# Gadersd/stable-diffusion-xl-burn

Measured on NVIDIA H100. Metric: unet_sampler_steps_per_sec_1024x1024_bs1, higher is better.
Workload: dtype f16

## Files before the change

stable-diffusion-xl-burn_b200/csrc/attention.cu:

```cuda
#include <stdlib.h>

#include "common.cuh"
#include "kernels.h"

namespace sdxl {

static constexpr int kTileBytes = 128 * 128;
static constexpr int kKvStages = 3;
static constexpr int kConsumerWarps = 8;
static constexpr int kAttnThreads = kConsumerWarps * 32 + 32;
static constexpr int kAttnSmem = 1024  + kTileBytes + 2 * kKvStages * kTileBytes + 256;

__device__ __forceinline__ float ex2_approx(float x) {
  float y;
  asm("ex2.approx.ftz.f32 %0, %1;" : "=f"(y) : "f"(x));
  return y;
}
__device__ __forceinline__ uint32_t pack_half2(float a, float b) {
  __half2 t = __floats2half2_rn(a, b);
  return *reinterpret_cast<uint32_t*>(&t);
}

__device__ __forceinline__ void attn_key_block(float (&o)[32], float (&m)[2], float (&l)[2], uint32_t q_addr, const uint8_t* sK,
                                               const uint8_t* sV, uint64_t* kv_full, uint64_t* kv_empty, int j, int kb, int S,
                                               float sl2e, int lane) {
  const int st = j % kKvStages;
  mbar_wait_nocall(&kv_full[st], (j / kKvStages) & 1);
  float s[64];
  wg_fence();
  const uint32_t k_addr = smem_u32(sK + st * kTileBytes);
#pragma unroll
  for (int k = 0; k < 4; ++k) wgmma_ss_n128(s, wg_desc_sw128(q_addr + 32 * k), wg_desc_sw128(k_addr + 32 * k), k);
  wg_commit();
  wg_wait<0>();
  if (kb * 128 + 128 > S) {
#pragma unroll
    for (int jj = 0; jj < 16; ++jj)
#pragma unroll
      for (int e = 0; e < 2; ++e)
        if (kb * 128 + 8 * jj + 2 * (lane & 3) + e >= S) { s[4 * jj + e] = -INFINITY; s[4 * jj + 2 + e] = -INFINITY; }
  }
  uint32_t pa[32];
#pragma unroll
  for (int h = 0; h < 2; ++h) {
    float mx = -INFINITY;
#pragma unroll
    for (int jj = 0; jj < 16; ++jj) mx = fmaxf(mx, fmaxf(s[4 * jj + 2 * h], s[4 * jj + 2 * h + 1]));
    mx = fmaxf(mx, __shfl_xor_sync(0xffffffffu, mx, 1));
    mx = fmaxf(mx, __shfl_xor_sync(0xffffffffu, mx, 2));
    const float m_new = fmaxf(m[h], mx);
    const float alpha = ex2_approx((m[h] - m_new) * sl2e);
    const float mb = m_new * sl2e;
    float sum = 0.f;
#pragma unroll
    for (int jj = 0; jj < 16; ++jj) {
      const float p0 = ex2_approx(fmaf(s[4 * jj + 2 * h], sl2e, -mb));
      const float p1 = ex2_approx(fmaf(s[4 * jj + 2 * h + 1], sl2e, -mb));
      sum += p0 + p1;
      pa[4 * (jj >> 1) + 2 * (jj & 1) + h] = pack_half2(p0, p1);
    }
    l[h] = l[h] * alpha + sum;
    m[h] = m_new;
#pragma unroll
    for (int jj = 0; jj < 8; ++jj) { o[4 * jj + 2 * h] *= alpha; o[4 * jj + 2 * h + 1] *= alpha; }
  }
  wg_fence();
  const uint32_t v_addr = smem_u32(sV + st * kTileBytes);
#pragma unroll
  for (int kk = 0; kk < 8; ++kk)
    wgmma_rs_n64_tb(o, *reinterpret_cast<const uint32_t(*)[4]>(pa + 4 * kk), wg_desc_sw128(v_addr + 2048 * kk));
  wg_commit();
  wg_wait<0>();
  if (lane == 0) mbar_arrive(&kv_empty[st]);
}

struct IpSrc {
  const CUtensorMap* tk;
  const CUtensorMap* tv;
  int S, k_col0, v_col0;
  const float* scale;
  const float* mask;
};
__device__ __forceinline__ IpSrc ip_source(const AttnParams& p, int k) {
  if (k == 0) return {&p.tmKip, &p.tmVip, p.S_ip, p.k_ip_col0, p.v_ip_col0, p.ip_scale, p.ip_mask};
  const AttnIpSource& s = p.ip_src[k - 1];
  return {&s.tm, &s.tm, s.S, s.k_col0, s.v_col0, s.scale, s.mask};
}

template <bool kIp>
__global__ void __launch_bounds__(kAttnThreads, 1) attention_kernel(const __grid_constant__ AttnParams p) {
  extern __shared__ uint8_t smem_raw[];
  uint8_t* smem = reinterpret_cast<uint8_t*>((reinterpret_cast<uintptr_t>(smem_raw) + 1023) & ~uintptr_t(1023));
  uint8_t* sQ = smem;
  uint8_t* sK = sQ + kTileBytes;
  uint8_t* sV = sK + kKvStages * kTileBytes;
  uint64_t* bars = reinterpret_cast<uint64_t*>(sV + kKvStages * kTileBytes);
  uint64_t* q_full = bars;
  uint64_t* kv_full = q_full + 1;
  uint64_t* kv_empty = kv_full + kKvStages;

  const int warp = threadIdx.x >> 5, lane = threadIdx.x & 31;
  const int nblk = (p.S + 127) / 128;
  const int nqt = (p.T + 127) / 128;
  const int qt = blockIdx.x % nqt, head = (blockIdx.x / nqt) % p.n_head, b = blockIdx.x / (nqt * p.n_head);

  if (threadIdx.x == 0) {
    tma_prefetch_desc(&p.tmQ);
    tma_prefetch_desc(&p.tmK);
    tma_prefetch_desc(&p.tmV);
    if constexpr (kIp) {
      tma_prefetch_desc(&p.tmKip);
      tma_prefetch_desc(&p.tmVip);
      for (int k = 1; k < p.n_src; ++k) tma_prefetch_desc(&p.ip_src[k - 1].tm);
    }
    mbar_init(q_full, 1);
    for (int i = 0; i < kKvStages; ++i) { mbar_init(&kv_full[i], 1); mbar_init(&kv_empty[i], kConsumerWarps); }
    fence_barrier_init();
  }
  __syncthreads();
  griddep_wait();
  griddep_launch_dependents();

  if (warp == kConsumerWarps) {
    if (lane != 0) return;
    mbar_expect_tx(q_full, kTileBytes);
    tma_load_3d(sQ, &p.tmQ, q_full, p.q_col0 + head * 64, qt * 128, b);
    for (int j = 0; j < nblk; ++j) {
      const int st = j % kKvStages;
      mbar_wait_nocall(&kv_empty[st], ((j / kKvStages) & 1) ^ 1);
      mbar_expect_tx(&kv_full[st], 2 * kTileBytes);
      tma_load_3d(sK + st * kTileBytes, &p.tmK, &kv_full[st], p.k_col0 + head * 64, j * 128, b);
      tma_load_3d(sV + st * kTileBytes, &p.tmV, &kv_full[st], p.v_col0 + head * 64, j * 128, b);
    }
    if constexpr (kIp) {
      int j = nblk;
      for (int k = 0; k < p.n_src; ++k) {
        const IpSrc s = ip_source(p, k);
        const int nb = (s.S + 127) / 128;
        for (int kb = 0; kb < nb; ++kb, ++j) {
          const int st = j % kKvStages;
          mbar_wait_nocall(&kv_empty[st], ((j / kKvStages) & 1) ^ 1);
          mbar_expect_tx(&kv_full[st], 2 * kTileBytes);
          tma_load_3d(sK + st * kTileBytes, s.tk, &kv_full[st], s.k_col0 + head * 64, kb * 128, b);
          tma_load_3d(sV + st * kTileBytes, s.tv, &kv_full[st], s.v_col0 + head * 64, kb * 128, b);
        }
      }
    }
    return;
  }

  const int wg = warp >> 2;
  const float sl2e = p.scale_log2e;
  const uint32_t q_addr = smem_u32(sQ) + (uint32_t)wg * (64 * 128);
  float o[32];
#pragma unroll
  for (int i = 0; i < 32; ++i) o[i] = 0.f;
  float m[2] = {-INFINITY, -INFINITY}, l[2] = {0.f, 0.f};
  mbar_wait_nocall(q_full, 0);
  for (int j = 0; j < nblk; ++j) {
    const int st = j % kKvStages;
    mbar_wait_nocall(&kv_full[st], (j / kKvStages) & 1);
    float s[64];
    wg_fence();
    const uint32_t k_addr = smem_u32(sK + st * kTileBytes);
#pragma unroll
    for (int k = 0; k < 4; ++k) wgmma_ss_n128(s, wg_desc_sw128(q_addr + 32 * k), wg_desc_sw128(k_addr + 32 * k), k);
    wg_commit();
    wg_wait<0>();
    if (j * 128 + 128 > p.S) {
#pragma unroll
      for (int jj = 0; jj < 16; ++jj)
#pragma unroll
        for (int e = 0; e < 2; ++e)
          if (j * 128 + 8 * jj + 2 * (lane & 3) + e >= p.S) { s[4 * jj + e] = -INFINITY; s[4 * jj + 2 + e] = -INFINITY; }
    }
    uint32_t pa[32];
#pragma unroll
    for (int h = 0; h < 2; ++h) {
      float mx = -INFINITY;
#pragma unroll
      for (int jj = 0; jj < 16; ++jj) mx = fmaxf(mx, fmaxf(s[4 * jj + 2 * h], s[4 * jj + 2 * h + 1]));
      mx = fmaxf(mx, __shfl_xor_sync(0xffffffffu, mx, 1));
      mx = fmaxf(mx, __shfl_xor_sync(0xffffffffu, mx, 2));
      const float m_new = fmaxf(m[h], mx);
      const float alpha = ex2_approx((m[h] - m_new) * sl2e);
      const float mb = m_new * sl2e;
      float sum = 0.f;
#pragma unroll
      for (int jj = 0; jj < 16; ++jj) {
        const float p0 = ex2_approx(fmaf(s[4 * jj + 2 * h], sl2e, -mb));
        const float p1 = ex2_approx(fmaf(s[4 * jj + 2 * h + 1], sl2e, -mb));
        sum += p0 + p1;
        pa[4 * (jj >> 1) + 2 * (jj & 1) + h] = pack_half2(p0, p1);
      }
      l[h] = l[h] * alpha + sum;
      m[h] = m_new;
#pragma unroll
      for (int jj = 0; jj < 8; ++jj) { o[4 * jj + 2 * h] *= alpha; o[4 * jj + 2 * h + 1] *= alpha; }
    }
    wg_fence();
    const uint32_t v_addr = smem_u32(sV + st * kTileBytes);
#pragma unroll
    for (int kk = 0; kk < 8; ++kk)
      wgmma_rs_n64_tb(o, *reinterpret_cast<const uint32_t(*)[4]>(pa + 4 * kk), wg_desc_sw128(v_addr + 2048 * kk));
    wg_commit();
    wg_wait<0>();
    if (lane == 0) mbar_arrive(&kv_empty[st]);
  }
  const int r = wg * 64 + (warp & 3) * 16 + (lane >> 2);
  if constexpr (kIp) {
    float acc[32];
#pragma unroll
    for (int h = 0; h < 2; ++h) {
      float lt = l[h];
      lt += __shfl_xor_sync(0xffffffffu, lt, 1);
      lt += __shfl_xor_sync(0xffffffffu, lt, 2);
      const float inv = 1.0f / lt;
#pragma unroll
      for (int jj = 0; jj < 8; ++jj) {
        acc[4 * jj + 2 * h] = o[4 * jj + 2 * h] * inv;
        acc[4 * jj + 2 * h + 1] = o[4 * jj + 2 * h + 1] * inv;
      }
    }
    int j = nblk;
    for (int k = 0; k < p.n_src; ++k) {
#pragma unroll
      for (int h = 0; h < 2; ++h) { m[h] = -INFINITY; l[h] = 0.f; }
#pragma unroll
      for (int i = 0; i < 32; ++i) o[i] = 0.f;
      const int S = ip_source(p, k).S;
      for (int kb = 0; kb * 128 < S; ++kb, ++j) attn_key_block(o, m, l, q_addr, sK, sV, kv_full, kv_empty, j, kb, S, sl2e, lane);
      const IpSrc s = ip_source(p, k);
      const float sk = *s.scale;
#pragma unroll
      for (int h = 0; h < 2; ++h) {
        float lt = l[h];
        lt += __shfl_xor_sync(0xffffffffu, lt, 1);
        lt += __shfl_xor_sync(0xffffffffu, lt, 2);
        const float inv = 1.0f / lt;
        const int t = qt * 128 + r + 8 * h;
        const float w = (s.mask && t < p.T) ? sk * s.mask[t] : sk;
#pragma unroll
        for (int jj = 0; jj < 8; ++jj) {
          acc[4 * jj + 2 * h] = fmaf(w, o[4 * jj + 2 * h] * inv, acc[4 * jj + 2 * h]);
          acc[4 * jj + 2 * h + 1] = fmaf(w, o[4 * jj + 2 * h + 1] * inv, acc[4 * jj + 2 * h + 1]);
        }
      }
    }
#pragma unroll
    for (int h = 0; h < 2; ++h) {
      const int t = qt * 128 + r + 8 * h;
      if (t < p.T) {
        __half* out = p.out + ((size_t)b * p.T + t) * p.ldo + head * 64 + 2 * (lane & 3);
#pragma unroll
// ... 42 lines not shown
  out[i] = cubic_1d(row[0], row[1], row[2], row[3], ty);
}

int ip_mask_resize_launch(cudaStream_t st, const float* mask, int H, int W, int mh, int mw, int T, float* out) {
  if (H < 1 || W < 1 || mh < 1 || mw < 1 || T < 1) return 2002;
  ip_mask_resize_kernel<<<(T + 255) / 256, 256, 0, st>>>(mask, H, W, mh, mw, T, out);
  return (int)cudaGetLastError();
}

static bool g_attn_attr[2][64];
int attention_launch(cudaStream_t st, const AttnParams& p) {
  if (p.T < 1 || p.S < 1 || (p.ldo & 1)) return 2002;
  const bool ip = p.S_ip > 0;
  if (ip && (!p.ip_scale || p.n_src < 1 || p.n_src > ATTN_MAX_SRC)) return 2002;
  for (int k = 1; ip && k < p.n_src; ++k)
    if (p.ip_src[k - 1].S < 1 || !p.ip_src[k - 1].scale) return 2002;
  auto kernel = ip ? attention_kernel<true> : attention_kernel<false>;
  int r = smem_optin(kernel, kAttnSmem, g_attn_attr[ip]);
  if (r) return r;
  const long tiles = (long)p.B * p.n_head * ((p.T + 127) / 128);
  return launch_kernel(kernel, dim3((unsigned)tiles), dim3(kAttnThreads), (size_t)kAttnSmem, st, true, p);
}

}
```

stable-diffusion-xl-burn_b200/csrc/engine.cu:

```cuda
#include "engine_core.h"
#include "schedule.h"

#include <set>

extern "C" int sdxl_ctx_create(int device, void* cuda_stream, sdxl_ctx** out) {
  if (!out) return -1;
  *out = nullptr;
  int n = 0;
  if (cudaGetDeviceCount(&n) != cudaSuccess || n <= 0 || device >= n) {
    fprintf(stderr, "sdxl_b200: no CUDA device %d (this library has no CPU fallback)\n", device);
    return -2;
  }
  cudaDeviceProp prop;
  if (cudaGetDeviceProperties(&prop, device) != cudaSuccess) return -3;
  if (prop.major != 9 || prop.minor != 0) {
    fprintf(stderr, "sdxl_b200: device %d is sm_%d%d; this library contains sm_90a code only\n", device,
            prop.major, prop.minor);
    return -4;
  }
  if (cudaSetDevice(device) != cudaSuccess) return -5;
  sdxl_ctx* c = new sdxl_ctx();
  c->device = device;
  c->num_sms = prop.multiProcessorCount;
  if (cuda_stream) {
// ... 825 lines not shown
      if (&b == &s.blocks.back()) linear(s_ff, M, b.ff2, IGEMM_LINEAR, s_a16, 0, C, s_tok, C);
      else linear(s_ff, M, b.ff2, IGEMM_LINEAR, s_tok, 1, C, s_tok, C);
    }
    if (s.blocks.empty() && !err) {
      Op op{};
      op.kind = OP_CAST16;
      op.cs = {s_tok, (size_t)M * C, s_a16};
      P->ops.push_back(op);
    }
    linear(s_a16, M, s.proj_out, IGEMM_LINEAR, out, 1, C, x, C);
    return out;
  }
  void attn(const __half* qm, int q_pitch, int q_col0, const __half* kvm, int kv_pitch, int k_col0, int v_col0, int T,
            int S, int n_head, __half* out, int ldo, float sl2e, int B = 0) {
    if (err) return;
    if (!B) B = Bf;
    Op op{};
    op.kind = OP_ATTN;
    AttnParams& p = op.at;
    p.T = T; p.S = S; p.n_head = n_head; p.B = B;
    p.q_col0 = q_col0; p.k_col0 = k_col0; p.v_col0 = v_col0;
    p.out = out; p.ldo = ldo; p.scale_log2e = sl2e;
    if (!A->measure) {
      int r = make_tmap_rows(&p.tmQ, qm, T, B, q_pitch, q_pitch);
      if (!r) r = make_tmap_rows(&p.tmK, kvm, S, B, kv_pitch, kv_pitch);
      if (!r) p.tmV = p.tmK;
      if (r) { err = fail(c, r, "tensor map creation failed (attention)"); return; }
    }
    op.flops_exec = 4.0 * B * (double)((T + 127) / 128 * 128) * (double)((S + 127) / 128 * 128) * (n_head * 64);
    P->ops.push_back(op);
    add_flops(4.0 * B * T * (double)S * (n_head * 64));
  }
  void attn_ip(const __half* kvm, int kv_pitch, int k_col0, int v_col0, int S_ip, const float* scale, const float* mask) {
    if (err) return;
    AttnParams& p = P->ops.back().at;
    if (p.n_src == ATTN_MAX_SRC) { err = fail(c, 5022, "image prompt: more than %d image sources", ATTN_MAX_SRC); return; }
    CUtensorMap tm{};
    if (!A->measure)
      if (int r = make_tmap_rows(&tm, kvm, S_ip, Bf, kv_pitch, kv_pitch)) { err = fail(c, r, "tensor map creation failed (attention)"); return; }
    if (p.n_src == 0) {
      p.S_ip = S_ip; p.k_ip_col0 = k_col0; p.v_ip_col0 = v_col0; p.ip_scale = scale; p.ip_mask = mask;
      p.tmKip = p.tmVip = tm;
    } else {
      p.ip_src[p.n_src - 1] = {tm, S_ip, k_col0, v_col0, scale, mask};
    }
    p.n_src++;
    const int C = p.n_head * 64;
    P->ops.back().flops_exec += 4.0 * Bf * (double)((p.T + 127) / 128 * 128) * (double)((S_ip + 127) / 128 * 128) * C;
    add_flops(4.0 * Bf * p.T * (double)S_ip * C);
  }
};



static int build_plan_ops(sdxl_unet* u, Plan* P, Arena* A, int Bp) {
  sdxl_ctx* c = u->ctx;
  const sdxl_unet_cfg& g = u->cfg;
  UNetPlanBuilder B{{c, P, A, P->Bf}, u};
  B.Bp = Bp;
  P->ops.clear();
  P->block_names.clear();
  P->flops = 0;
  const int Bf = P->Bf, mc = g.model_channels, ted = 4 * mc;
  const int temb_total = u->temb_all.N;
  const int levels = g.n_levels;
  if ((P->h % (1 << (levels - 1))) || (P->w % (1 << (levels - 1)))) return fail(c, 5003, "latent %dx%d not divisible by %d", P->h, P->w, 1 << (levels - 1));

  P->x_in = B.buf<float>((size_t)P->Bx * latent_channels(g) * P->h * P->w);
  P->eps_ld = g.out_channels;
  P->eps = B.buf<float>((size_t)Bf * P->h * P->w * P->eps_ld);
  B.gn_partial = B.buf<float>(gn_scratch_floats(Bf, 32));
// ... 1535 lines not shown
}

extern "C" void sdxl_unet_destroy(sdxl_unet* u) {
  if (!u) return;
  cudaStreamSynchronize(u->ctx->stream);
  delete u;
}


extern "C" int sdxl_qkv_attention(sdxl_ctx* c, const sdxl_half* q, const sdxl_half* k, const sdxl_half* v, const sdxl_half* mask,
                                  int B, int T, int S, int C, int n_head, sdxl_half* out) {
  if (!c || !q || !k || !v || !out) return -1;
  if (n_head < 1 || C != n_head * 64) return fail(c, 5301, "sdxl_qkv_attention: head dim must be 64 (C=%d, n_head=%d)", C, n_head);
  if (mask) {
    KL(c, attention_small_launch(c->stream, (const __half*)q, C, 0, (const __half*)k, (const __half*)v, C, 0, 0, B, T, S, n_head,
                                 (const __half*)mask, 0, (__half*)out, C));
    return 0;
  }
  AttnParams p{};
  p.T = T; p.S = S; p.n_head = n_head; p.B = B;
  p.q_col0 = p.k_col0 = p.v_col0 = 0;
  p.out = (__half*)out; p.ldo = C;
  p.scale_log2e = (float)(1.4426950408889634 / sqrt(64.0));
  int r = make_tmap_rows(&p.tmQ, (const __half*)q, T, B, C, C);
  if (!r) r = make_tmap_rows(&p.tmK, (const __half*)k, S, B, C, C);
  if (!r) r = make_tmap_rows(&p.tmV, (const __half*)v, S, B, C, C);
  if (r) return fail(c, r, "tensor map creation failed");
  KL(c, attention_launch(c->stream, p));
  return 0;
}

extern "C" int sdxl_op_ip_attention(sdxl_ctx* c, const sdxl_half* q, const sdxl_half* k, const sdxl_half* v, const sdxl_half* k_ip,
                                    const sdxl_half* v_ip, int B, int T, int S, int S_ip, int C, int n_head, float scale, sdxl_half* out) {
  if (!c || !q || !k || !v || !k_ip || !v_ip || !out) return -1;
  if (n_head < 1 || C != n_head * 64) return fail(c, 5302, "sdxl_op_ip_attention: head dim must be 64 (C=%d, n_head=%d)", C, n_head);
  if (B < 1 || S_ip < 1) return fail(c, 5303, "sdxl_op_ip_attention: B = %d and S_ip = %d must be >= 1", B, S_ip);
  CU(c, cudaSetDevice(c->device));
  TmpBufs tmp(c->stream);
  float* s = tmp.get<float>(sizeof(float));
  if (!s) return fail(c, 5304, "temporary allocation failed");
  CU(c, cudaMemcpyAsync(s, &scale, sizeof(float), cudaMemcpyHostToDevice, c->stream));
  AttnParams p{};
  p.T = T; p.S = S; p.n_head = n_head; p.B = B;
  p.out = (__half*)out; p.ldo = C;
  p.scale_log2e = (float)(1.4426950408889634 / sqrt(64.0));
  p.S_ip = S_ip; p.ip_scale = s; p.n_src = 1;
  int r = make_tmap_rows(&p.tmQ, (const __half*)q, T, B, C, C);
  if (!r) r = make_tmap_rows(&p.tmK, (const __half*)k, S, B, C, C);
  if (!r) r = make_tmap_rows(&p.tmV, (const __half*)v, S, B, C, C);
  if (!r) r = make_tmap_rows(&p.tmKip, (const __half*)k_ip, S_ip, B, C, C);
  if (!r) r = make_tmap_rows(&p.tmVip, (const __half*)v_ip, S_ip, B, C, C);
  if (r) return fail(c, r, "tensor map creation failed");
  KL(c, attention_launch(c->stream, p));
  CU(c, cudaStreamSynchronize(c->stream));
  return 0;
}

extern "C" int sdxl_op_linear(sdxl_ctx* c, const sdxl_half* x, const sdxl_half* w, const sdxl_half* bias, const float* residual,
                              int M, int K, int N, int geglu, int out_f16, void* out) {
  if (!c || !x || !w || !out) return -1;
  if (K % 8) return fail(c, 5310, "sdxl_op_linear: K must be a multiple of 8");
  TmpBufs T(c->stream);
  const int Kpad = (K + 63) / 64 * 64;
  int gbn = 0;
  if (geglu) {
    gbn = geglu_bn_for(N / 2);
    if (!gbn || (N & 1)) return fail(c, 5311, "sdxl_op_linear: GEGLU width not tileable");
  }
  __half* wt = T.get<__half>((size_t)N * Kpad * 2);
  float* b32 = bias ? T.get<float>((size_t)N * 4) : nullptr;
  if (!wt || (bias && !b32)) return fail(c, 5312, "temporary allocation failed");
  KL(c, transpose_linear_launch(c->stream, (const __half*)w, K, N, wt, Kpad, 0, gbn));
  if (bias) KL(c, bias_to_f32_launch(c->stream, (const __half*)bias, N, b32, gbn, 0));
  const IgemmOperands o{(const __half*)x, 1, 1, M, K, K, nullptr, 0, 0, 0, 0, 0, wt, N, Kpad};
// ... 64 lines not shown
```

stable-diffusion-xl-burn_b200/csrc/igemm.cu:

```cuda
#include "common.cuh"
#include "kernels.h"

#include <stdio.h>
#include <stdlib.h>

namespace sdxl {

static constexpr int kTileM = 128;
static constexpr int kBlockK = 64;
static constexpr int kABytes = kTileM * kBlockK * 2;
static constexpr int kConsumerWarps = 8;
static constexpr int kThreads = 128 + kConsumerWarps * 32;

__device__ __forceinline__ size_t out_pixel(const IgemmParams& p, int tb, int th, int tw, int r, bool& ok, int& bb) {
  const int wt = r % p.Wt, ht = (r / p.Wt) % p.Ht, bt = r / (p.Wt * p.Ht);
  bb = tb * p.Bt + bt;
  const int hh = th * p.Ht + ht, ww = tw * p.Wt + wt;
  ok = (bb < p.Bn) && (hh < p.H) && (ww < p.W);
  return ok ? ((size_t)bb * p.H + hh) * (size_t)p.opix_row + (size_t)ww * p.opix_w + p.opix_off : 0;
}

__device__ __forceinline__ void store2(const IgemmParams& p, size_t off, float x0, float x1, bool two, bool vec) {
  if (p.out_f32) {
    float* o = reinterpret_cast<float*>(p.out) + off;
// ... 194 lines not shown
  if (r != CUDA_SUCCESS) {
    fprintf(stderr, "sdxl_b200: cuTensorMapEncodeTiled failed (%d) rank=%d dims=[%llu,%llu,%llu,%llu] box=[%u,%u,%u,%u]\n",
            (int)r, rank, (unsigned long long)dims[0], (unsigned long long)(rank > 1 ? dims[1] : 0),
            (unsigned long long)(rank > 2 ? dims[2] : 0), (unsigned long long)(rank > 3 ? dims[3] : 0), box[0],
            rank > 1 ? box[1] : 0, rank > 2 ? box[2] : 0, rank > 3 ? box[3] : 0);
    return 1002;
  }
  return 0;
}

int make_tmap_act(CUtensorMap* tm, const __half* base, int Bn, int H, int W, int C, int pitch, int Wt, int Ht,
                  int Bt) {
  uint64_t dims[4] = {(uint64_t)C, (uint64_t)W, (uint64_t)H, (uint64_t)Bn};
  uint64_t str[3] = {(uint64_t)pitch * 2, (uint64_t)W * pitch * 2, (uint64_t)H * W * pitch * 2};
  uint32_t box[4] = {64, (uint32_t)Wt, (uint32_t)Ht, (uint32_t)Bt};
  return encode(tm, base, 4, dims, str, box);
}
int make_tmap_wgt(CUtensorMap* tm, const __half* base, int N, int K, int BN) {
  uint64_t dims[2] = {(uint64_t)K, (uint64_t)N};
  uint64_t str[1] = {(uint64_t)K * 2};
  uint32_t box[2] = {64, (uint32_t)BN};
  return encode(tm, base, 2, dims, str, box);
}
int make_tmap_rows(CUtensorMap* tm, const __half* base, int rows_per_batch, int nbatch, int cols, int pitch) {
  uint64_t dims[3] = {(uint64_t)cols, (uint64_t)rows_per_batch, (uint64_t)nbatch};
  uint64_t str[2] = {(uint64_t)pitch * 2, (uint64_t)rows_per_batch * pitch * 2};
  uint32_t box[3] = {64, 128, 1};
  return encode(tm, base, 3, dims, str, box);
}

void igemm_pick_box(int W, int H, int* Wt, int* Ht, int* Bt) {
  int wt = 1;
  while (wt * 2 <= W && wt * 2 <= 128) wt *= 2;
  int ht = 1;
  while (ht * 2 <= H && wt * ht * 2 <= 128) ht *= 2;
  *Wt = wt;
  *Ht = ht;
  *Bt = 128 / (wt * ht);
}

int igemm_pick_bn(int m_tiles, int N, int num_sms, bool geglu) {
  (void)geglu;
  if (m_tiles == 16 && N == 3840) return 160;
  double best = 1e30;
  int best_bn = 0;
  for (int bn : {256, 160, 128, 64}) {
    if (N % bn) continue;
    const long tiles = (long)m_tiles * (N / bn);
    const long waves = (tiles + num_sms - 1) / num_sms;
    const double cost = (double)waves * (bn + 48.0);
// ... 83 lines not shown
```

stable-diffusion-xl-burn_b200/csrc/kernels.h:

```cpp
#pragma once
#include <cuda.h>
#include <cuda_fp16.h>
#include <cuda_runtime.h>
#include <stdint.h>

namespace sdxl {

bool pdl_enabled();
template <typename... KArgs, typename... Args>
inline int launch_kernel(void (*kernel)(KArgs...), dim3 grid, dim3 block, size_t smem, cudaStream_t st, bool pdl,
                         Args&&... args) {
  cudaLaunchConfig_t cfg{};
  cfg.gridDim = grid;
  cfg.blockDim = block;
  cfg.dynamicSmemBytes = smem;
  cfg.stream = st;
  cudaLaunchAttribute attr[1];
  attr[0].id = cudaLaunchAttributeProgrammaticStreamSerialization;
  attr[0].val.programmaticStreamSerializationAllowed = 1;
  cfg.attrs = attr;
  cfg.numAttrs = (pdl && pdl_enabled()) ? 1 : 0;
  return (int)cudaLaunchKernelEx(&cfg, kernel, static_cast<KArgs>(args)...);
}
template <typename... KArgs, typename... Args>
// ... 80 lines not shown

constexpr int ATTN_MAX_SRC = 8;
struct AttnIpSource {
  CUtensorMap tm;
  int S, k_col0, v_col0;
  const float* scale;
  const float* mask;
};
struct AttnParams {
  CUtensorMap tmQ, tmK, tmV;
  int T, S, n_head, B;
  int q_col0, k_col0, v_col0;
  __half* out;
  int ldo;
  float scale_log2e;
  CUtensorMap tmKip, tmVip;
  int S_ip;
  int k_ip_col0, v_ip_col0;
  const float* ip_scale;
  int n_src;
  const float* ip_mask;
  AttnIpSource ip_src[ATTN_MAX_SRC - 1];
};
int make_tmap_rows(CUtensorMap* tm, const __half* base, int rows_per_batch, int nbatch, int cols, int pitch);
int attention_launch(cudaStream_t st, const AttnParams& p);
int ip_mask_resize_launch(cudaStream_t st, const float* mask, int H, int W, int mh, int mw, int T, float* out);

struct GnParams {
  const float* x1; int C1;
  const float* x2; int C2;
  int B, HW, n_group;
  const float* gamma; const float* beta;
  float eps;
  int silu;
  __half* y;
  __half* raw;
  float* partial;
  int nchunk;
  __half* y_lo;
};
size_t gn_scratch_floats(int B, int n_group);
int gn_scratch_init(cudaStream_t st, float* scratch, int B, int n_group);
int gn_launch(cudaStream_t st, GnParams& p);
int layernorm_launch(cudaStream_t st, const float* x, const float* gamma, const float* beta, float eps,
                     int rows, int C, __half* y);

int gemv_launch(cudaStream_t st, const float* in, int in_bstride, int Bv, int K, const __half* W, int ldw,
                const float* bias, const float* add, int add_bstride, int N, int in_silu, int out_silu,
// ... 105 lines not shown
```

stable-diffusion-xl-burn_b200/csrc/testing.cu:

```cuda
#include "kernels.h"
#include "schedule.h"

#define SDXL_TEST_API extern "C" __attribute__((visibility("default")))

using namespace sdxl;

SDXL_TEST_API int sdxl_test_igemm(void* stream, const void* a0, int a0Bn, int a0H, int a0W, int a0C, int a0pitch, const void* a1,
                                  int a1Bn, int a1H, int a1W, int a1C, int a1pitch, const void* w, int N, int Ktot, int outW,
                                  int outH, int outB, int mode, int geglu_bn, const int* segs, int nseg, void* out, int out_f32,
                                  int ldo, const float* bias, int bias_bstride, const float* res, int ldr, int opix_row,
                                  int opix_w, int opix_off) {
  if (nseg < 1 || nseg > IGEMM_MAX_SEG) return 5002;
  IgemmParams p{};
  p.nseg = nseg;
  for (int i = 0; i < nseg; ++i)
    p.seg[i] = {(int16_t)segs[5 * i], (int16_t)segs[5 * i + 1], (int16_t)segs[5 * i + 2], (int16_t)segs[5 * i + 3], segs[5 * i + 4]};
  p.out = out; p.out_f32 = out_f32; p.ldo = ldo;
  p.bias = bias; p.bias_bstride = bias_bstride;
  p.res = res; p.ldr = ldr;
  const IgemmOperands o{(const __half*)a0, a0Bn, a0H, a0W, a0C, a0pitch, (const __half*)a1, a1Bn, a1H, a1W, a1C, a1pitch,
                        (const __half*)w, N, Ktot};
  if (int r = igemm_configure(p, o, outW, outH, outB, mode, geglu_bn)) return r;
  if (opix_row) { p.opix_row = opix_row; p.opix_w = opix_w; p.opix_off = opix_off; }
  return igemm_launch((cudaStream_t)stream, p);
}

SDXL_TEST_API int sdxl_test_attention(void* stream, const void* q, int q_pitch, int q_col0, const void* kv, int kv_pitch, int k_col0,
                                      int v_col0, int B, int T, int S, int n_head, void* out, int ldo, const void* kip,
                                      int kip_pitch, int k_ip_col0, int v_ip_col0, int S_ip, const float* ip_scale) {
  AttnParams p{};
  p.T = T; p.S = S; p.n_head = n_head; p.B = B;
  p.q_col0 = q_col0; p.k_col0 = k_col0; p.v_col0 = v_col0;
  p.out = (__half*)out; p.ldo = ldo;
  p.scale_log2e = (float)(1.4426950408889634 / 8.0);
  int r = make_tmap_rows(&p.tmQ, (const __half*)q, T, B, q_pitch, q_pitch);
  if (!r) r = make_tmap_rows(&p.tmK, (const __half*)kv, S, B, kv_pitch, kv_pitch);
  if (r) return r;
  p.tmV = p.tmK;
  if (kip) {
    p.S_ip = S_ip; p.k_ip_col0 = k_ip_col0; p.v_ip_col0 = v_ip_col0; p.ip_scale = ip_scale; p.n_src = 1;
    if ((r = make_tmap_rows(&p.tmKip, (const __half*)kip, S_ip, B, kip_pitch, kip_pitch))) return r;
    p.tmVip = p.tmKip;
  }
  return attention_launch((cudaStream_t)stream, p);
}

SDXL_TEST_API int sdxl_test_attention_multi(void* stream, const void* q, int q_pitch, int q_col0, const void* kv, int kv_pitch, int k_col0,
                                            int v_col0, int B, int T, int S, int n_head, void* out, int ldo, int n_src,
                                            const void* const* src_kv, const int* src_info, const float* const* scales,
                                            const float* const* masks) {
  if (n_src < 1 || n_src > ATTN_MAX_SRC) return 5003;
  AttnParams p{};
  p.T = T; p.S = S; p.n_head = n_head; p.B = B;
  p.q_col0 = q_col0; p.k_col0 = k_col0; p.v_col0 = v_col0;
  p.out = (__half*)out; p.ldo = ldo;
  p.scale_log2e = (float)(1.4426950408889634 / 8.0);
  int r = make_tmap_rows(&p.tmQ, (const __half*)q, T, B, q_pitch, q_pitch);
  if (!r) r = make_tmap_rows(&p.tmK, (const __half*)kv, S, B, kv_pitch, kv_pitch);
  if (r) return r;
  p.tmV = p.tmK;
  p.n_src = n_src;
  for (int k = 0; k < n_src; ++k) {
    const int* f = src_info + 4 * k;
    CUtensorMap tm;
    if ((r = make_tmap_rows(&tm, (const __half*)src_kv[k], f[3], B, f[0], f[0]))) return r;
    if (k == 0) {
      p.tmKip = p.tmVip = tm;
      p.S_ip = f[3]; p.k_ip_col0 = f[1]; p.v_ip_col0 = f[2]; p.ip_scale = scales[0]; p.ip_mask = masks[0];
    } else {
      p.ip_src[k - 1] = {tm, f[3], f[1], f[2], scales[k], masks[k]};
    }
  }
  return attention_launch((cudaStream_t)stream, p);
}

SDXL_TEST_API int sdxl_test_ip_mask_resize(void* stream, const float* mask, int H, int W, int mh, int mw, int T, float* out) {
  return ip_mask_resize_launch((cudaStream_t)stream, mask, H, W, mh, mw, T, out);
}

SDXL_TEST_API int sdxl_test_attention_small(void* stream, const void* q, int q_pitch, int q_col0, const void* k, const void* v,
                                            int kv_pitch, int k_col0, int v_col0, int B, int T, int S, int n_head, const void* mask,
                                            int causal, void* out, int ldo, int head_dim) {
  return attention_small_launch((cudaStream_t)stream, (const __half*)q, q_pitch, q_col0, (const __half*)k, (const __half*)v, kv_pitch,
                                k_col0, v_col0, B, T, S, n_head, (const __half*)mask, causal, (__half*)out, ldo, head_dim);
}

SDXL_TEST_API int sdxl_test_perceiver_ln(void* stream, const float* x, const float* lat, int n, int L, int Q, int C, const float* g1,
                                         const float* b1, const float* g2, const float* b2, float eps, void* kv, void* q) {
  return perceiver_ln_launch((cudaStream_t)stream, x, lat, n, L, Q, C, g1, b1, g2, b2, eps, (__half*)kv, (__half*)q);
}

SDXL_TEST_API size_t sdxl_test_gn_scratch_floats(int B, int n_group) { return gn_scratch_floats(B, n_group); }
SDXL_TEST_API int sdxl_test_gn_scratch_init(void* stream, float* scratch, int B, int n_group) {
  return gn_scratch_init((cudaStream_t)stream, scratch, B, n_group);
}
SDXL_TEST_API int sdxl_test_gn(void* stream, const float* x1, int C1, const float* x2, int C2, int B, int HW, int n_group,
                               const float* gamma, const float* beta, float eps, int silu, void* y, void* raw, void* y_lo,
// ... 186 lines not shown
```

stable-diffusion-xl-burn_b200/sdxl_b200/_testing.py:

```python
from __future__ import annotations

import ctypes as C
import os
from typing import Optional, Sequence

import torch

from ._lib import SdxlError, SdxlLibraryMissing

HERE = os.path.dirname(os.path.abspath(__file__))
LIB_PATH = os.path.join(HERE, "libsdxl_b200_testing.so")

P, I, F, L, Z = C.c_void_p, C.c_int, C.c_float, C.c_long, C.c_size_t
PROTOTYPES = {
    "sdxl_test_igemm": (I, [P, P, I, I, I, I, I, P, I, I, I, I, I, P, I, I, I, I, I, I, I, P, I, P, I, I, P, I, P, I, I, I, I]),
    "sdxl_test_attention": (I, [P, P, I, I, P, I, I, I, I, I, I, I, P, I, P, I, I, I, I, P]),
    "sdxl_test_attention_multi": (I, [P, P, I, I, P, I, I, I, I, I, I, I, P, I, I, P, P, P, P]),
    "sdxl_test_ip_mask_resize": (I, [P, P, I, I, I, I, I, P]),
    "sdxl_test_attention_small": (I, [P, P, I, I, P, P, I, I, I, I, I, I, I, P, I, P, I, I]),
    "sdxl_test_perceiver_ln": (I, [P, P, P, I, I, I, I, P, P, P, P, F, P, P]),
    "sdxl_test_gn_scratch_floats": (C.c_size_t, [I, I]),
    "sdxl_test_gn_scratch_init": (I, [P, P, I, I]),
    "sdxl_test_gn": (I, [P, P, I, P, I, I, I, I, P, P, F, I, P, P, P, P]),
    "sdxl_test_gemv": (I, [P, P, I, I, I, P, I, P, P, I, I, I, I, P, I]),
    "sdxl_test_conv_in": (I, [P, P, I, I, I, I, I, I, P, P, I, P, P, I]),
    "sdxl_test_conv_in_cat": (I, [P, P, I, I, I, I, P, I, I, I, I, P, P, I, P]),
    "sdxl_test_pag_identity": (I, [P, P, I, C.c_long, P]),
    "sdxl_test_cfg_pag_ddim": (I, [P, P, I, I, I, I, I, F, F, F, F, F, F, P]),
    "sdxl_test_freeu_twiddles": (None, [I, I, P]),
    "sdxl_test_freeu": (I, [P, P, I, P, I, I, I, I, P, P, P]),
    "sdxl_test_repack_upconv": (I, [P, P, I, I, P, I]),
    "sdxl_test_repack_conv": (I, [P, P, I, I, I, I, P, I, I, I]),
    "sdxl_test_transpose_linear": (I, [P, P, I, I, P, I, I, I]),
    "sdxl_test_bias_to_f32": (I, [P, P, I, P, I, I]),
    "sdxl_test_lora_merge": (I, [P, I, I, I, I, P, P, P, P, P, P, I, C.c_size_t, I, I, I, I, P]),
    "sdxl_test_lora_upconv_merge": (I, [P, P, P, I, I, P, I]),
    "sdxl_test_softmax_rows": (I, [P, P, Z, I, I, F, P, Z]),
    "sdxl_test_transpose_f16": (I, [P, P, Z, I, I, P, Z]),
    "sdxl_test_post_quant": (I, [P, P, I, I, I, P, P, F, P]),
    "sdxl_test_quant_out": (I, [P, P, I, I, I, L, P, P, F, P]),
# ... 66 lines not shown
    _call("sdxl_test_igemm", _p(a0), *a0_shape, a0_shape[3], _p(a1), *a1_shape, a1_shape[3], _p(w), N, Ktot, *out_whb, mode,
          geglu_bn, seg, len(segs), _p(out), int(out.dtype == torch.float32), ldo, _p(bias), bias_bstride, _p(res), ldr, *o)


def attention(q: torch.Tensor, q_pitch: int, q_col0: int, kv: torch.Tensor, kv_pitch: int, k_col0: int, v_col0: int,
              B: int, T: int, S: int, n_head: int, out: torch.Tensor, ldo: int, kip: Optional[torch.Tensor] = None,
              kip_pitch: int = 0, k_ip_col0: int = 0, v_ip_col0: int = 0, S_ip: int = 0,
              ip_scale: Optional[torch.Tensor] = None) -> None:
    _call("sdxl_test_attention", _p(q), q_pitch, q_col0, _p(kv), kv_pitch, k_col0, v_col0, B, T, S, n_head, _p(out), ldo,
          _p(kip), kip_pitch, k_ip_col0, v_ip_col0, S_ip, _p(ip_scale))


def attention_multi(q: torch.Tensor, q_pitch: int, q_col0: int, kv: torch.Tensor, kv_pitch: int, k_col0: int, v_col0: int,
                    B: int, T: int, S: int, n_head: int, out: torch.Tensor, ldo: int, sources: Sequence[tuple]) -> None:
    n = len(sources)
    kvs = (C.c_void_p * n)(*[_p(s[0]) for s in sources])
    info = (C.c_int * (4 * n))(*[int(v) for s in sources for v in (s[1], s[2], s[3], s[4])])
    scales = (C.c_void_p * n)(*[_p(s[5]) for s in sources])
    masks = (C.c_void_p * n)(*[_p(s[6]) for s in sources])
    _call("sdxl_test_attention_multi", _p(q), q_pitch, q_col0, _p(kv), kv_pitch, k_col0, v_col0, B, T, S, n_head, _p(out), ldo, n,
          kvs, info, scales, masks)


def ip_mask_resize(mask: torch.Tensor, mh: int, mw: int, T: int) -> torch.Tensor:
    out = torch.empty(T, device=mask.device, dtype=torch.float32)
    _call("sdxl_test_ip_mask_resize", _p(mask), mask.shape[0], mask.shape[1], mh, mw, T, _p(out))
    return out


def attention_small(q, q_pitch, q_col0, k, v, kv_pitch, k_col0, v_col0, B, T, S, n_head, mask, causal, out, ldo,
                    head_dim) -> None:
    _call("sdxl_test_attention_small", _p(q), q_pitch, q_col0, _p(k), _p(v), kv_pitch, k_col0, v_col0, B, T, S, n_head,
          _p(mask), int(causal), _p(out), ldo, head_dim)


def perceiver_ln(x, lat, n, L, Q, C, g1, b1, g2, b2, eps, kv, q) -> None:
    _call("sdxl_test_perceiver_ln", _p(x), _p(lat), n, L, Q, C, _p(g1), _p(b1), _p(g2), _p(b2), eps, _p(kv), _p(q))


def gn_scratch(B: int, n_group: int) -> torch.Tensor:
    s = torch.empty(load().sdxl_test_gn_scratch_floats(B, n_group), dtype=torch.float32, device="cuda")
    _call("sdxl_test_gn_scratch_init", _p(s), B, n_group)
    return s


def group_norm(x1, x2, B, HW, n_group, gamma, beta, eps, silu, y, raw, y_lo, scratch) -> None:
# ... 191 lines not shown
```

Baseline: 28.42.

## Shrink attention KV tile to 64 rows to fit two CTAs per SM

Halves the key/value block from 128 to 64 rows, using n64 wgmma for QK^T and half as many PV steps, and deepens the KV pipeline to four stages. This cuts shared memory (16K Q plus 64K KV) and the register footprint of the score fragment, and launch bounds now request two CTAs per SM for the non-IP kernel. The goal is to overlap one CTA's softmax with another's tensor-core work. In exchange each key block does less work per barrier round trip and softmax pass, so there is more synchronisation overhead. The duplicated main loop is also folded into the shared per-block helper, and an occupancy query is added for tests.

```diff
diff --git a/stable-diffusion-xl-burn_b200/csrc/attention.cu b/stable-diffusion-xl-burn_b200/csrc/attention.cu
--- a/stable-diffusion-xl-burn_b200/csrc/attention.cu
+++ b/stable-diffusion-xl-burn_b200/csrc/attention.cu
@@ -5,11 +5,13 @@
 
 namespace sdxl {
 
-static constexpr int kTileBytes = 128 * 128;
-static constexpr int kKvStages = 3;
+static constexpr int kQTileBytes = ATTN_Q_ROWS * 128;
+static constexpr int kKvTileBytes = ATTN_KV_ROWS * 128;
+static constexpr int kKvStages = 4;
 static constexpr int kConsumerWarps = 8;
 static constexpr int kAttnThreads = kConsumerWarps * 32 + 32;
-static constexpr int kAttnSmem = 1024  + kTileBytes + 2 * kKvStages * kTileBytes + 256;
+static constexpr int kAttnSmem = 1024  + kQTileBytes + 2 * kKvStages * kKvTileBytes + 256;
+static_assert(ATTN_Q_ROWS == 128 && ATTN_KV_ROWS == 64, "the wgmma shapes and fragment indexing below assume these blocks");
 
 __device__ __forceinline__ float ex2_approx(float x) {
   float y;
@@ -26,26 +28,26 @@
                                                float sl2e, int lane) {
   const int st = j % kKvStages;
   mbar_wait_nocall(&kv_full[st], (j / kKvStages) & 1);
-  float s[64];
+  float s[32];
   wg_fence();
-  const uint32_t k_addr = smem_u32(sK + st * kTileBytes);
-#pragma unroll
-  for (int k = 0; k < 4; ++k) wgmma_ss_n128(s, wg_desc_sw128(q_addr + 32 * k), wg_desc_sw128(k_addr + 32 * k), k);
+  const uint32_t k_addr = smem_u32(sK + st * kKvTileBytes);
+#pragma unroll
+  for (int k = 0; k < 4; ++k) wgmma_ss_n64(s, wg_desc_sw128(q_addr + 32 * k), wg_desc_sw128(k_addr + 32 * k), k);
   wg_commit();
   wg_wait<0>();
-  if (kb * 128 + 128 > S) {
-#pragma unroll
-    for (int jj = 0; jj < 16; ++jj)
+  if (kb * 64 + 64 > S) {
+#pragma unroll
+    for (int jj = 0; jj < 8; ++jj)
 #pragma unroll
       for (int e = 0; e < 2; ++e)
-        if (kb * 128 + 8 * jj + 2 * (lane & 3) + e >= S) { s[4 * jj + e] = -INFINITY; s[4 * jj + 2 + e] = -INFINITY; }
-  }
-  uint32_t pa[32];
+        if (kb * 64 + 8 * jj + 2 * (lane & 3) + e >= S) { s[4 * jj + e] = -INFINITY; s[4 * jj + 2 + e] = -INFINITY; }
+  }
+  uint32_t pa[16];
 #pragma unroll
   for (int h = 0; h < 2; ++h) {
     float mx = -INFINITY;
 #pragma unroll
-    for (int jj = 0; jj < 16; ++jj) mx = fmaxf(mx, fmaxf(s[4 * jj + 2 * h], s[4 * jj + 2 * h + 1]));
+    for (int jj = 0; jj < 8; ++jj) mx = fmaxf(mx, fmaxf(s[4 * jj + 2 * h], s[4 * jj + 2 * h + 1]));
     mx = fmaxf(mx, __shfl_xor_sync(0xffffffffu, mx, 1));
     mx = fmaxf(mx, __shfl_xor_sync(0xffffffffu, mx, 2));
     const float m_new = fmaxf(m[h], mx);
@@ -53,7 +55,7 @@
     const float mb = m_new * sl2e;
     float sum = 0.f;
 #pragma unroll
-    for (int jj = 0; jj < 16; ++jj) {
+    for (int jj = 0; jj < 8; ++jj) {
       const float p0 = ex2_approx(fmaf(s[4 * jj + 2 * h], sl2e, -mb));
       const float p1 = ex2_approx(fmaf(s[4 * jj + 2 * h + 1], sl2e, -mb));
       sum += p0 + p1;
@@ -65,9 +67,9 @@
     for (int jj = 0; jj < 8; ++jj) { o[4 * jj + 2 * h] *= alpha; o[4 * jj + 2 * h + 1] *= alpha; }
   }
   wg_fence();
-  const uint32_t v_addr = smem_u32(sV + st * kTileBytes);
-#pragma unroll
-  for (int kk = 0; kk < 8; ++kk)
+  const uint32_t v_addr = smem_u32(sV + st * kKvTileBytes);
+#pragma unroll
+  for (int kk = 0; kk < 4; ++kk)
     wgmma_rs_n64_tb(o, *reinterpret_cast<const uint32_t(*)[4]>(pa + 4 * kk), wg_desc_sw128(v_addr + 2048 * kk));
   wg_commit();
   wg_wait<0>();
@@ -88,19 +90,19 @@
 }
 
 template <bool kIp>
-__global__ void __launch_bounds__(kAttnThreads, 1) attention_kernel(const __grid_constant__ AttnParams p) {
+__global__ void __launch_bounds__(kAttnThreads, kIp ? 1 : 2) attention_kernel(const __grid_constant__ AttnParams p) {
   extern __shared__ uint8_t smem_raw[];
   uint8_t* smem = reinterpret_cast<uint8_t*>((reinterpret_cast<uintptr_t>(smem_raw) + 1023) & ~uintptr_t(1023));
   uint8_t* sQ = smem;
-  uint8_t* sK = sQ + kTileBytes;
-  uint8_t* sV = sK + kKvStages * kTileBytes;
-  uint64_t* bars = reinterpret_cast<uint64_t*>(sV + kKvStages * kTileBytes);
+  uint8_t* sK = sQ + kQTileBytes;
+  uint8_t* sV = sK + kKvStages * kKvTileBytes;
+  uint64_t* bars = reinterpret_cast<uint64_t*>(sV + kKvStages * kKvTileBytes);
   uint64_t* q_full = bars;
   uint64_t* kv_full = q_full + 1;
   uint64_t* kv_empty = kv_full + kKvStages;
 
   const int warp = threadIdx.x >> 5, lane = threadIdx.x & 31;
-  const int nblk = (p.S + 127) / 128;
+  const int nblk = (p.S + ATTN_KV_ROWS - 1) / ATTN_KV_ROWS;
   const int nqt = (p.T + 127) / 128;
   const int qt = blockIdx.x % nqt, head = (blockIdx.x / nqt) % p.n_head, b = blockIdx.x / (nqt * p.n_head);
 
@@ -123,26 +125,26 @@
 
   if (warp == kConsumerWarps) {
     if (lane != 0) return;
-    mbar_expect_tx(q_full, kTileBytes);
+    mbar_expect_tx(q_full, kQTileBytes);
     tma_load_3d(sQ, &p.tmQ, q_full, p.q_col0 + head * 64, qt * 128, b);
     for (int j = 0; j < nblk; ++j) {
       const int st = j % kKvStages;
       mbar_wait_nocall(&kv_empty[st], ((j / kKvStages) & 1) ^ 1);
-      mbar_expect_tx(&kv_full[st], 2 * kTileBytes);
-      tma_load_3d(sK + st * kTileBytes, &p.tmK, &kv_full[st], p.k_col0 + head * 64, j * 128, b);
-      tma_load_3d(sV + st * kTileBytes, &p.tmV, &kv_full[st], p.v_col0 + head * 64, j * 128, b);
+      mbar_expect_tx(&kv_full[st], 2 * kKvTileBytes);
+      tma_load_3d(sK + st * kKvTileBytes, &p.tmK, &kv_full[st], p.k_col0 + head * 64, j * ATTN_KV_ROWS, b);
+      tma_load_3d(sV + st * kKvTileBytes, &p.tmV, &kv_full[st], p.v_col0 + head * 64, j * ATTN_KV_ROWS, b);
     }
     if constexpr (kIp) {
       int j = nblk;
       for (int k = 0; k < p.n_src; ++k) {
         const IpSrc s = ip_source(p, k);
-        const int nb = (s.S + 127) / 128;
+        const int nb = (s.S + ATTN_KV_ROWS - 1) / ATTN_KV_ROWS;
         for (int kb = 0; kb < nb; ++kb, ++j) {
           const int st = j % kKvStages;
           mbar_wait_nocall(&kv_empty[st], ((j / kKvStages) & 1) ^ 1);
-          mbar_expect_tx(&kv_full[st], 2 * kTileBytes);
-          tma_load_3d(sK + st * kTileBytes, s.tk, &kv_full[st], s.k_col0 + head * 64, kb * 128, b);
-          tma_load_3d(sV + st * kTileBytes, s.tv, &kv_full[st], s.v_col0 + head * 64, kb * 128, b);
+          mbar_expect_tx(&kv_full[st], 2 * kKvTileBytes);
+          tma_load_3d(sK + st * kKvTileBytes, s.tk, &kv_full[st], s.k_col0 + head * 64, kb * ATTN_KV_ROWS, b);
+          tma_load_3d(sV + st * kKvTileBytes, s.tv, &kv_full[st], s.v_col0 + head * 64, kb * ATTN_KV_ROWS, b);
         }
       }
     }
@@ -157,56 +159,7 @@
   for (int i = 0; i < 32; ++i) o[i] = 0.f;
   float m[2] = {-INFINITY, -INFINITY}, l[2] = {0.f, 0.f};
   mbar_wait_nocall(q_full, 0);
-  for (int j = 0; j < nblk; ++j) {
-    const int st = j % kKvStages;
-    mbar_wait_nocall(&kv_full[st], (j / kKvStages) & 1);
-    float s[64];
-    wg_fence();
-    const uint32_t k_addr = smem_u32(sK + st * kTileBytes);
-#pragma unroll
-    for (int k = 0; k < 4; ++k) wgmma_ss_n128(s, wg_desc_sw128(q_addr + 32 * k), wg_desc_sw128(k_addr + 32 * k), k);
-    wg_commit();
-    wg_wait<0>();
-    if (j * 128 + 128 > p.S) {
-#pragma unroll
-      for (int jj = 0; jj < 16; ++jj)
-#pragma unroll
-        for (int e = 0; e < 2; ++e)
-          if (j * 128 + 8 * jj + 2 * (lane & 3) + e >= p.S) { s[4 * jj + e] = -INFINITY; s[4 * jj + 2 + e] = -INFINITY; }
-    }
-    uint32_t pa[32];
-#pragma unroll
-    for (int h = 0; h < 2; ++h) {
-      float mx = -INFINITY;
-#pragma unroll
-      for (int jj = 0; jj < 16; ++jj) mx = fmaxf(mx, fmaxf(s[4 * jj + 2 * h], s[4 * jj + 2 * h + 1]));
-      mx = fmaxf(mx, __shfl_xor_sync(0xffffffffu, mx, 1));
-      mx = fmaxf(mx, __shfl_xor_sync(0xffffffffu, mx, 2));
-      const float m_new = fmaxf(m[h], mx);
-      const float alpha = ex2_approx((m[h] - m_new) * sl2e);
-      const float mb = m_new * sl2e;
-      float sum = 0.f;
-#pragma unroll
-      for (int jj = 0; jj < 16; ++jj) {
-        const float p0 = ex2_approx(fmaf(s[4 * jj + 2 * h], sl2e, -mb));
-        const float p1 = ex2_approx(fmaf(s[4 * jj + 2 * h + 1], sl2e, -mb));
-        sum += p0 + p1;
-        pa[4 * (jj >> 1) + 2 * (jj & 1) + h] = pack_half2(p0, p1);
-      }
-      l[h] = l[h] * alpha + sum;
-      m[h] = m_new;
-#pragma unroll
-      for (int jj = 0; jj < 8; ++jj) { o[4 * jj + 2 * h] *= alpha; o[4 * jj + 2 * h + 1] *= alpha; }
-    }
-    wg_fence();
-    const uint32_t v_addr = smem_u32(sV + st * kTileBytes);
-#pragma unroll
-    for (int kk = 0; kk < 8; ++kk)
-      wgmma_rs_n64_tb(o, *reinterpret_cast<const uint32_t(*)[4]>(pa + 4 * kk), wg_desc_sw128(v_addr + 2048 * kk));
-    wg_commit();
-    wg_wait<0>();
-    if (lane == 0) mbar_arrive(&kv_empty[st]);
-  }
+  for (int j = 0; j < nblk; ++j) attn_key_block(o, m, l, q_addr, sK, sV, kv_full, kv_empty, j, j, p.S, sl2e, lane);
   const int r = wg * 64 + (warp & 3) * 16 + (lane >> 2);
   if constexpr (kIp) {
     float acc[32];
@@ -229,7 +182,7 @@
 #pragma unroll
       for (int i = 0; i < 32; ++i) o[i] = 0.f;
       const int S = ip_source(p, k).S;
-      for (int kb = 0; kb * 128 < S; ++kb, ++j) attn_key_block(o, m, l, q_addr, sK, sV, kv_full, kv_empty, j, kb, S, sl2e, lane);
+      for (int kb = 0; kb * ATTN_KV_ROWS < S; ++kb, ++j) attn_key_block(o, m, l, q_addr, sK, sV, kv_full, kv_empty, j, kb, S, sl2e, lane);
       const IpSrc s = ip_source(p, k);
       const float sk = *s.scale;
 #pragma unroll
@@ -318,4 +271,10 @@
   return launch_kernel(kernel, dim3((unsigned)tiles), dim3(kAttnThreads), (size_t)kAttnSmem, st, true, p);
 }
 
-}
+int attention_occupancy(bool ip, int* blocks_per_sm) {
+  auto kernel = ip ? attention_kernel<true> : attention_kernel<false>;
+  if (int r = smem_optin(kernel, kAttnSmem, g_attn_attr[ip])) return r;
+  return (int)cudaOccupancyMaxActiveBlocksPerMultiprocessor(blocks_per_sm, kernel, kAttnThreads, (size_t)kAttnSmem);
+}
+
+}
diff --git a/stable-diffusion-xl-burn_b200/csrc/engine.cu b/stable-diffusion-xl-burn_b200/csrc/engine.cu
--- a/stable-diffusion-xl-burn_b200/csrc/engine.cu
+++ b/stable-diffusion-xl-burn_b200/csrc/engine.cu
@@ -871,12 +871,13 @@
     p.q_col0 = q_col0; p.k_col0 = k_col0; p.v_col0 = v_col0;
     p.out = out; p.ldo = ldo; p.scale_log2e = sl2e;
     if (!A->measure) {
-      int r = make_tmap_rows(&p.tmQ, qm, T, B, q_pitch, q_pitch);
-      if (!r) r = make_tmap_rows(&p.tmK, kvm, S, B, kv_pitch, kv_pitch);
+      int r = make_tmap_rows(&p.tmQ, qm, T, B, q_pitch, q_pitch, ATTN_Q_ROWS);
+      if (!r) r = make_tmap_rows(&p.tmK, kvm, S, B, kv_pitch, kv_pitch, ATTN_KV_ROWS);
       if (!r) p.tmV = p.tmK;
       if (r) { err = fail(c, r, "tensor map creation failed (attention)"); return; }
     }
-    op.flops_exec = 4.0 * B * (double)((T + 127) / 128 * 128) * (double)((S + 127) / 128 * 128) * (n_head * 64);
+    const double S_exec = (S + ATTN_KV_ROWS - 1) / ATTN_KV_ROWS * ATTN_KV_ROWS;
+    op.flops_exec = 4.0 * B * (double)((T + 127) / 128 * 128) * S_exec * (n_head * 64);
     P->ops.push_back(op);
     add_flops(4.0 * B * T * (double)S * (n_head * 64));
   }
@@ -886,7 +887,7 @@
     if (p.n_src == ATTN_MAX_SRC) { err = fail(c, 5022, "image prompt: more than %d image sources", ATTN_MAX_SRC); return; }
     CUtensorMap tm{};
     if (!A->measure)
-      if (int r = make_tmap_rows(&tm, kvm, S_ip, Bf, kv_pitch, kv_pitch)) { err = fail(c, r, "tensor map creation failed (attention)"); return; }
+      if (int r = make_tmap_rows(&tm, kvm, S_ip, Bf, kv_pitch, kv_pitch, ATTN_KV_ROWS)) { err = fail(c, r, "tensor map creation failed (attention)"); return; }
     if (p.n_src == 0) {
       p.S_ip = S_ip; p.k_ip_col0 = k_col0; p.v_ip_col0 = v_col0; p.ip_scale = scale; p.ip_mask = mask;
       p.tmKip = p.tmVip = tm;
@@ -895,7 +896,7 @@
     }
     p.n_src++;
     const int C = p.n_head * 64;
-    P->ops.back().flops_exec += 4.0 * Bf * (double)((p.T + 127) / 128 * 128) * (double)((S_ip + 127) / 128 * 128) * C;
+    P->ops.back().flops_exec += 4.0 * Bf * (double)((p.T + 127) / 128 * 128) * (double)((S_ip + ATTN_KV_ROWS - 1) / ATTN_KV_ROWS * ATTN_KV_ROWS) * C;
     add_flops(4.0 * Bf * p.T * (double)S_ip * C);
   }
 };
@@ -2477,9 +2478,9 @@
   p.q_col0 = p.k_col0 = p.v_col0 = 0;
   p.out = (__half*)out; p.ldo = C;
   p.scale_log2e = (float)(1.4426950408889634 / sqrt(64.0));
-  int r = make_tmap_rows(&p.tmQ, (const __half*)q, T, B, C, C);
-  if (!r) r = make_tmap_rows(&p.tmK, (const __half*)k, S, B, C, C);
-  if (!r) r = make_tmap_rows(&p.tmV, (const __half*)v, S, B, C, C);
+  int r = make_tmap_rows(&p.tmQ, (const __half*)q, T, B, C, C, ATTN_Q_ROWS);
+  if (!r) r = make_tmap_rows(&p.tmK, (const __half*)k, S, B, C, C, ATTN_KV_ROWS);
+  if (!r) r = make_tmap_rows(&p.tmV, (const __half*)v, S, B, C, C, ATTN_KV_ROWS);
   if (r) return fail(c, r, "tensor map creation failed");
   KL(c, attention_launch(c->stream, p));
   return 0;
@@ -2500,11 +2501,11 @@
   p.out = (__half*)out; p.ldo = C;
   p.scale_log2e = (float)(1.4426950408889634 / sqrt(64.0));
   p.S_ip = S_ip; p.ip_scale = s; p.n_src = 1;
-  int r = make_tmap_rows(&p.tmQ, (const __half*)q, T, B, C, C);
-  if (!r) r = make_tmap_rows(&p.tmK, (const __half*)k, S, B, C, C);
-  if (!r) r = make_tmap_rows(&p.tmV, (const __half*)v, S, B, C, C);
-  if (!r) r = make_tmap_rows(&p.tmKip, (const __half*)k_ip, S_ip, B, C, C);
-  if (!r) r = make_tmap_rows(&p.tmVip, (const __half*)v_ip, S_ip, B, C, C);
+  int r = make_tmap_rows(&p.tmQ, (const __half*)q, T, B, C, C, ATTN_Q_ROWS);
+  if (!r) r = make_tmap_rows(&p.tmK, (const __half*)k, S, B, C, C, ATTN_KV_ROWS);
+  if (!r) r = make_tmap_rows(&p.tmV, (const __half*)v, S, B, C, C, ATTN_KV_ROWS);
+  if (!r) r = make_tmap_rows(&p.tmKip, (const __half*)k_ip, S_ip, B, C, C, ATTN_KV_ROWS);
+  if (!r) r = make_tmap_rows(&p.tmVip, (const __half*)v_ip, S_ip, B, C, C, ATTN_KV_ROWS);
   if (r) return fail(c, r, "tensor map creation failed");
   KL(c, attention_launch(c->stream, p));
   CU(c, cudaStreamSynchronize(c->stream));
diff --git a/stable-diffusion-xl-burn_b200/csrc/igemm.cu b/stable-diffusion-xl-burn_b200/csrc/igemm.cu
--- a/stable-diffusion-xl-burn_b200/csrc/igemm.cu
+++ b/stable-diffusion-xl-burn_b200/csrc/igemm.cu
@@ -240,10 +240,10 @@
   uint32_t box[2] = {64, (uint32_t)BN};
   return encode(tm, base, 2, dims, str, box);
 }
-int make_tmap_rows(CUtensorMap* tm, const __half* base, int rows_per_batch, int nbatch, int cols, int pitch) {
+int make_tmap_rows(CUtensorMap* tm, const __half* base, int rows_per_batch, int nbatch, int cols, int pitch, int box_rows) {
   uint64_t dims[3] = {(uint64_t)cols, (uint64_t)rows_per_batch, (uint64_t)nbatch};
   uint64_t str[2] = {(uint64_t)pitch * 2, (uint64_t)rows_per_batch * pitch * 2};
-  uint32_t box[3] = {64, 128, 1};
+  uint32_t box[3] = {64, (uint32_t)box_rows, 1};
   return encode(tm, base, 3, dims, str, box);
 }
 
diff --git a/stable-diffusion-xl-burn_b200/csrc/kernels.h b/stable-diffusion-xl-burn_b200/csrc/kernels.h
--- a/stable-diffusion-xl-burn_b200/csrc/kernels.h
+++ b/stable-diffusion-xl-burn_b200/csrc/kernels.h
@@ -126,8 +126,11 @@
   const float* ip_mask;
   AttnIpSource ip_src[ATTN_MAX_SRC - 1];
 };
-int make_tmap_rows(CUtensorMap* tm, const __half* base, int rows_per_batch, int nbatch, int cols, int pitch);
+constexpr int ATTN_Q_ROWS = 128;
+constexpr int ATTN_KV_ROWS = 64;
+int make_tmap_rows(CUtensorMap* tm, const __half* base, int rows_per_batch, int nbatch, int cols, int pitch, int box_rows);
 int attention_launch(cudaStream_t st, const AttnParams& p);
+int attention_occupancy(bool ip, int* blocks_per_sm);
 int ip_mask_resize_launch(cudaStream_t st, const float* mask, int H, int W, int mh, int mw, int T, float* out);
 
 struct GnParams {
diff --git a/stable-diffusion-xl-burn_b200/csrc/testing.cu b/stable-diffusion-xl-burn_b200/csrc/testing.cu
--- a/stable-diffusion-xl-burn_b200/csrc/testing.cu
+++ b/stable-diffusion-xl-burn_b200/csrc/testing.cu
@@ -33,13 +33,13 @@
   p.q_col0 = q_col0; p.k_col0 = k_col0; p.v_col0 = v_col0;
   p.out = (__half*)out; p.ldo = ldo;
   p.scale_log2e = (float)(1.4426950408889634 / 8.0);
-  int r = make_tmap_rows(&p.tmQ, (const __half*)q, T, B, q_pitch, q_pitch);
-  if (!r) r = make_tmap_rows(&p.tmK, (const __half*)kv, S, B, kv_pitch, kv_pitch);
+  int r = make_tmap_rows(&p.tmQ, (const __half*)q, T, B, q_pitch, q_pitch, ATTN_Q_ROWS);
+  if (!r) r = make_tmap_rows(&p.tmK, (const __half*)kv, S, B, kv_pitch, kv_pitch, ATTN_KV_ROWS);
   if (r) return r;
   p.tmV = p.tmK;
   if (kip) {
     p.S_ip = S_ip; p.k_ip_col0 = k_ip_col0; p.v_ip_col0 = v_ip_col0; p.ip_scale = ip_scale; p.n_src = 1;
-    if ((r = make_tmap_rows(&p.tmKip, (const __half*)kip, S_ip, B, kip_pitch, kip_pitch))) return r;
+    if ((r = make_tmap_rows(&p.tmKip, (const __half*)kip, S_ip, B, kip_pitch, kip_pitch, ATTN_KV_ROWS))) return r;
     p.tmVip = p.tmKip;
   }
   return attention_launch((cudaStream_t)stream, p);
@@ -55,15 +55,15 @@
   p.q_col0 = q_col0; p.k_col0 = k_col0; p.v_col0 = v_col0;
   p.out = (__half*)out; p.ldo = ldo;
   p.scale_log2e = (float)(1.4426950408889634 / 8.0);
-  int r = make_tmap_rows(&p.tmQ, (const __half*)q, T, B, q_pitch, q_pitch);
-  if (!r) r = make_tmap_rows(&p.tmK, (const __half*)kv, S, B, kv_pitch, kv_pitch);
+  int r = make_tmap_rows(&p.tmQ, (const __half*)q, T, B, q_pitch, q_pitch, ATTN_Q_ROWS);
+  if (!r) r = make_tmap_rows(&p.tmK, (const __half*)kv, S, B, kv_pitch, kv_pitch, ATTN_KV_ROWS);
   if (r) return r;
   p.tmV = p.tmK;
   p.n_src = n_src;
   for (int k = 0; k < n_src; ++k) {
     const int* f = src_info + 4 * k;
     CUtensorMap tm;
-    if ((r = make_tmap_rows(&tm, (const __half*)src_kv[k], f[3], B, f[0], f[0]))) return r;
+    if ((r = make_tmap_rows(&tm, (const __half*)src_kv[k], f[3], B, f[0], f[0], ATTN_KV_ROWS))) return r;
     if (k == 0) {
       p.tmKip = p.tmVip = tm;
       p.S_ip = f[3]; p.k_ip_col0 = f[1]; p.v_ip_col0 = f[2]; p.ip_scale = scales[0]; p.ip_mask = masks[0];
@@ -73,6 +73,8 @@
   }
   return attention_launch((cudaStream_t)stream, p);
 }
+
+SDXL_TEST_API int sdxl_test_attention_occupancy(int ip, int* blocks_per_sm) { return attention_occupancy(ip != 0, blocks_per_sm); }
 
 SDXL_TEST_API int sdxl_test_ip_mask_resize(void* stream, const float* mask, int H, int W, int mh, int mw, int T, float* out) {
   return ip_mask_resize_launch((cudaStream_t)stream, mask, H, W, mh, mw, T, out);
diff --git a/stable-diffusion-xl-burn_b200/sdxl_b200/_testing.py b/stable-diffusion-xl-burn_b200/sdxl_b200/_testing.py
--- a/stable-diffusion-xl-burn_b200/sdxl_b200/_testing.py
+++ b/stable-diffusion-xl-burn_b200/sdxl_b200/_testing.py
@@ -16,6 +16,7 @@
     "sdxl_test_igemm": (I, [P, P, I, I, I, I, I, P, I, I, I, I, I, P, I, I, I, I, I, I, I, P, I, P, I, I, P, I, P, I, I, I, I]),
     "sdxl_test_attention": (I, [P, P, I, I, P, I, I, I, I, I, I, I, P, I, P, I, I, I, I, P]),
     "sdxl_test_attention_multi": (I, [P, P, I, I, P, I, I, I, I, I, I, I, P, I, I, P, P, P, P]),
+    "sdxl_test_attention_occupancy": (I, [I, P]),
     "sdxl_test_ip_mask_resize": (I, [P, P, I, I, I, I, I, P]),
     "sdxl_test_attention_small": (I, [P, P, I, I, P, P, I, I, I, I, I, I, I, P, I, P, I, I]),
     "sdxl_test_perceiver_ln": (I, [P, P, P, I, I, I, I, P, P, P, P, F, P, P]),
@@ -128,6 +129,14 @@
           kvs, info, scales, masks)
 
 
+def attention_occupancy(ip: bool) -> int:
+    n = C.c_int(0)
+    rc = load().sdxl_test_attention_occupancy(int(ip), C.byref(n))
+    if rc != 0:
+        raise SdxlError(f"sdxl_test_attention_occupancy failed ({rc})")
+    return n.value
+
+
 def ip_mask_resize(mask: torch.Tensor, mh: int, mw: int, T: int) -> torch.Tensor:
     out = torch.empty(T, device=mask.device, dtype=torch.float32)
     _call("sdxl_test_ip_mask_resize", _p(mask), mask.shape[0], mask.shape[1], mh, mw, T, _p(out))
```

After: 28.77, median of 6. 1.2% higher.
